# 3dhumangan/3DHumanGAN

Hardware: AMD Instinct MI355X
Metric: generator images/sec at 512^2 (higher is better)
Workload: dtype f32 in/out, f32 accumulate; contractions field f16x2 / synthesis f16x2 (x2 = f16 product + block-scaled fp6 cross terms, x3 = three f16/bf16 products); 1 GPU; BASELINE cfg 3: MAP3DBN512 generator-only forward, 512x512 out, 96x96 rays x 64 samples, hidden 256, batch 16/GPU, mixed, random-init weights, procedural SMPL-like pose; global_batch=16, parallelism=batch-sharded replicas x1 (no collective)

## Files before the change

### 3dhumangan_amd/csrc/geo_features.hip

```cpp
#include "common.hpp"

namespace {

constexpr int kThreads = 512;
constexpr int kPts = 4;
constexpr int kJoints = 24;
constexpr int kChunk = 64;
constexpr int kCand = 6;

typedef float f2 __attribute__((ext_vector_type(2)));
typedef float f4 __attribute__((ext_vector_type(4)));
typedef float f16v __attribute__((ext_vector_type(16)));
typedef unsigned u4 __attribute__((ext_vector_type(4)));
typedef int i4 __attribute__((ext_vector_type(4)));
typedef _Float16 half8 __attribute__((ext_vector_type(8)));
typedef _Float16 half2v __attribute__((ext_vector_type(2)));

__device__ __forceinline__ unsigned split2_f16(float a, float b, unsigned& lo) {
    const half2v h2 = __builtin_convertvector(f2{a, b}, half2v);
    lo = __builtin_bit_cast(unsigned, __builtin_convertvector(f2{a - (float)h2.x, b - (float)h2.y}, half2v));
    return __builtin_bit_cast(unsigned, h2);
}

__device__ __forceinline__ float sqdist_exact(float px, float py, float pz, float vx, float vy, float vz) {
    const float dx = __fsub_rn(px, vx), dy = __fsub_rn(py, vy), dz = __fsub_rn(pz, vz);
    return __fadd_rn(__fadd_rn(__fmul_rn(dx, dx), __fmul_rn(dy, dy)), __fmul_rn(dz, dz));
}

template <bool SORTED>
__device__ __forceinline__ void refine(const f4* vx4, const f4* vy4, const f4* vz4, const i4* ids4, int v4_begin, int v4_end,
                                       float px, float py, float pz, float& best, int& bi) {
#pragma clang loop unroll(disable)
    for (int v4 = v4_begin; v4 < v4_end; ++v4) {
        const f4 X = vx4[v4], Y = vy4[v4], Z = vz4[v4];
        const float d0 = sqdist_exact(px, py, pz, X.x, Y.x, Z.x);
        const float d1 = sqdist_exact(px, py, pz, X.y, Y.y, Z.y);
        const float d2 = sqdist_exact(px, py, pz, X.z, Y.z, Z.z);
        const float d3 = sqdist_exact(px, py, pz, X.w, Y.w, Z.w);
        if constexpr (SORTED) {
            const i4 I = ids4[v4];
            unsigned long long key = ((unsigned long long)__float_as_uint(best) << 32) | (unsigned)bi;
            const unsigned long long k0 = ((unsigned long long)__float_as_uint(d0) << 32) | (unsigned)I.x;
            const unsigned long long k1 = ((unsigned long long)__float_as_uint(d1) << 32) | (unsigned)I.y;
            const unsigned long long k2 = ((unsigned long long)__float_as_uint(d2) << 32) | (unsigned)I.z;
            const unsigned long long k3 = ((unsigned long long)__float_as_uint(d3) << 32) | (unsigned)I.w;
            key = k0 < key ? k0 : key;
            key = k1 < key ? k1 : key;
            key = k2 < key ? k2 : key;
            key = k3 < key ? k3 : key;
            best = __uint_as_float((unsigned)(key >> 32));
            bi = (int)(unsigned)key;
        } else {
            if (d0 < best) { best = d0; bi = v4 * 4 + 0; }
            if (d1 < best) { best = d1; bi = v4 * 4 + 1; }
            if (d2 < best) { best = d2; bi = v4 * 4 + 2; }
            if (d3 < best) { best = d3; bi = v4 * 4 + 3; }
        }
    }
}

template <bool FEATURES, bool SORTED>
__global__ __launch_bounds__(kThreads) void geo_features_kernel(
    const float* __restrict__ points, const float* __restrict__ joints, const float* __restrict__ vertices,
    const float* __restrict__ tpose, const float* __restrict__ vertex_ik, float* __restrict__ geo,
    int32_t* __restrict__ nn_index, int64_t N, int V, int Vpad, int geo_stride, int legacy_mode, int tile_S, int tile_Wr,
    int tiles_x, int tiles_y) {
    extern __shared__ __attribute__((aligned(16))) float smem[];
    float* vx = smem;
    float* vy = smem + Vpad;
    float* vz = smem + 2 * Vpad;
    int* vid = reinterpret_cast<int*>(smem + 3 * Vpad);
    float* jl = smem + (SORTED ? 4 : 3) * Vpad;
    unsigned* v2max_bits = reinterpret_cast<unsigned*>(jl + kJoints * 3);
    const int b = blockIdx.y;
    const int t = threadIdx.x;
    const float* __restrict__ vb = vertices + (int64_t)b * V * 3;
    const f4* __restrict__ ws = reinterpret_cast<const f4*>(vertices) + (int64_t)b * (Vpad + Vpad / kChunk);
    const f4* __restrict__ bounds = ws + Vpad;
    if (t == 0) *v2max_bits = 0u;
    __syncthreads();
    float v2 = 0.f;
    for (int i = t; i < Vpad; i += kThreads) {
        const bool ok = SORTED ? true : i < V;
        float x, y, z;
        if constexpr (SORTED) {
            const f4 q = ws[i];
            x = q.x; y = q.y; z = q.z;
            vid[i] = __float_as_int(q.w);
        } else {
            x = ok ? vb[i * 3 + 0] : 3.0e18f; y = ok ? vb[i * 3 + 1] : 3.0e18f; z = ok ? vb[i * 3 + 2] : 3.0e18f;
        }
        vx[i] = x; vy[i] = y; vz[i] = z;
        if (x < 1.0e18f) v2 = fmaxf(v2, x * x + y * y + z * z);
    }
    atomicMax(v2max_bits, __float_as_uint(v2));
    if (FEATURES && t < kJoints * 3) jl[t] = joints[(int64_t)b * kJoints * 3 + t];
    __syncthreads();
    const float v2max = __uint_as_float(*v2max_bits);

    const int lane = t & 63, m = lane & 31, hh = lane >> 5;
    const int64_t wave_id = (int64_t)blockIdx.x * (kThreads / 64) + (t >> 6);
    const int64_t wbase = wave_id * 256;
    int64_t tile_base = 0;
    bool tile_ok = true;
    if (tile_S > 0) {
        const int tiles_s = tile_S / 4;
        const int sz = (int)(wave_id % tiles_s);
        const int64_t pxy = wave_id / tiles_s;
        const int px_ = (int)(pxy % tiles_x), py_ = (int)(pxy / tiles_x);
        tile_ok = py_ < tiles_y;
        tile_base = (((int64_t)py_ * 8) * tile_Wr + px_ * 8) * tile_S + sz * 4;
    }
    auto point_of = [&](int i) -> int64_t {
        if (tile_S == 0) return wbase + i;
        if (!tile_ok) return N;
        const int ri = i >> 2;
        return tile_base + ((int64_t)(ri >> 3) * tile_Wr + (ri & 7)) * tile_S + (i & 3);
    };
    float px[kPts], py[kPts], pz[kPts], best[kPts];
    int bi[kPts];
#pragma unroll
    for (int k = 0; k < kPts; ++k) {
        const int64_t n = point_of((4 * hh + k) * 32 + m);
        const bool ok = n < N;
        const float* p = points + ((int64_t)b * N + (ok ? n : 0)) * 3;
        px[k] = p[0]; py[k] = p[1]; pz[k] = p[2];
        best[k] = 3.4e38f;
        bi[k] = 0;
    }
    const f4* vx4 = reinterpret_cast<const f4*>(vx);
    const f4* vy4 = reinterpret_cast<const f4*>(vy);
    const f4* vz4 = reinterpret_cast<const f4*>(vz);
    const i4* vid4 = reinterpret_cast<const i4*>(vid);

    half8 bfrag[8];
#pragma unroll
    for (int j = 0; j < 8; ++j) {
        const int k = j & 3;
        const float ox = __shfl_xor(px[k], 32, 64), oy = __shfl_xor(py[k], 32, 64), oz = __shfl_xor(pz[k], 32, 64);
        const bool own = (j >> 2) == hh;
        const float x = -2.f * (own ? px[k] : ox), y = -2.f * (own ? py[k] : oy), z = -2.f * (own ? pz[k] : oz);
        unsigned lo01, lo23;
        const unsigned hi01 = split2_f16(x, y, lo01), hi23 = split2_f16(z, 1.f, lo23);
        bfrag[j] = __builtin_bit_cast(half8, u4{hi01, hi23, hh ? 0u : lo01, hh ? 0u : lo23});
    }
    float run[kPts], tol[kPts], cval[kPts][kCand];
    float sk[kPts], sb[kPts];
    unsigned long long cid[kPts];
    int ncand[kPts];
#pragma unroll
    for (int k = 0; k < kPts; ++k) {
        const float p2 = px[k] * px[k] + py[k] * py[k] + pz[k] * pz[k];
        const float S = p2 + v2max;
        tol[k] = (S < 1.0e4f) ? 3.0517578e-5f * S : 3.0e38f;
        sb[k] = 3.f * tol[k] + p2;
        run[k] = 3.0e38f;
        sk[k] = 3.0e18f;
        cid[k] = 0ull;
        ncand[k] = 0;
#pragma unroll
        for (int q = 0; q < kCand; ++q) cval[k][q] = 3.4e38f;
    }
    const int n_chunks = Vpad / kChunk;
    int seed = -1;
    if constexpr (SORTED) {
        float sx = (px[0] + px[1]) + (px[2] + px[3]), sy = (py[0] + py[1]) + (py[2] + py[3]), sz = (pz[0] + pz[1]) + (pz[2] + pz[3]);
#pragma unroll
        for (int d = 32; d >= 1; d >>= 1) {
            sx += __shfl_xor(sx, d, 64); sy += __shfl_xor(sy, d, 64); sz += __shfl_xor(sz, d, 64);
        }
        sx *= 1.f / 256.f; sy *= 1.f / 256.f; sz *= 1.f / 256.f;
        float bd = 3.4e38f;
        int bc = 0;
        for (int c0 = lane; c0 < n_chunks; c0 += 64) {
            const f4 cb = bounds[c0];
            const float dx = sx - cb.x, dy = sy - cb.y, dz = sz - cb.z;
            const float d2 = dx * dx + dy * dy + dz * dz;
            if (d2 < bd) { bd = d2; bc = c0; }
        }
#pragma unroll
        for (int d = 32; d >= 1; d >>= 1) {
            const float od = __shfl_xor(bd, d, 64);
            const int oc = __shfl_xor(bc, d, 64);
            if (od < bd || (od == bd && oc < bc)) { bd = od; bc = oc; }
        }
        seed = __builtin_amdgcn_readfirstlane(bc);
    }
#pragma clang loop unroll(disable)
    for (int it = 0; it < n_chunks; ++it) {
        const int c = !SORTED ? it : it == 0 ? seed : (it <= seed ? it - 1 : it);
        if constexpr (SORTED) {
            const f4 cb = bounds[c];
            bool need = false;
#pragma unroll
            for (int k = 0; k < kPts; ++k) {
                const float dx = px[k] - cb.x, dy = py[k] - cb.y, dz = pz[k] - cb.z;
                const float d2 = dx * dx + dy * dy + dz * dz;
                const float reach = cb.w + sk[k];
                need |= d2 <= reach * reach;
            }
            if (__builtin_amdgcn_ballot_w64(need) == 0ull) continue;
        }
        float cmv[8];
#pragma unroll
        for (int j = 0; j < 8; ++j) cmv[j] = 3.4e38f;
#pragma unroll
        for (int tile = 0; tile < kChunk / 32; ++tile) {
            const int v = c * kChunk + tile * 32 + m;
            const bool real = v < V;
            const float x = real ? vx[v] : 0.f, y = real ? vy[v] : 0.f, z = real ? vz[v] : 0.f;
            const float w = real ? fmaf(z, z, fmaf(y, y, x * x)) : 6.0e4f;
            unsigned lo01, lo23;
            const unsigned hi01 = split2_f16(x, y, lo01), hi23 = split2_f16(z, w, lo23);
            const half8 afrag = __builtin_bit_cast(half8, hh ? u4{lo01, lo23, 0u, 0u} : u4{hi01, hi23, hi01, hi23});
#pragma unroll
            for (int j = 0; j < 8; ++j) {
                const f16v zero = {0.f, 0.f, 0.f, 0.f, 0.f, 0.f, 0.f, 0.f, 0.f, 0.f, 0.f, 0.f, 0.f, 0.f, 0.f, 0.f};
                const f16v d = __builtin_amdgcn_mfma_f32_32x32x16_f16(afrag, bfrag[j], zero, 0, 0, 0);
                float mn = cmv[j];
#pragma unroll
                for (int r = 0; r < 16; r += 2) mn = fminf(fminf(mn, d[r]), d[r + 1]);
                cmv[j] = mn;
            }
        }
        float cm[kPts];
#pragma unroll
        for (int k = 0; k < kPts; ++k) {
            const float lo_set = fminf(cmv[k], __shfl_xor(cmv[k], 32, 64));
            const float hi_set = fminf(cmv[4 + k], __shfl_xor(cmv[4 + k], 32, 64));
            cm[k] = hh ? hi_set : lo_set;
        }
#pragma unroll
        for (int k = 0; k < kPts; ++k) {
            if (cm[k] <= run[k] + tol[k]) {
#pragma unroll
                for (int q = 0; q < kCand - 1; ++q) cval[k][q] = cval[k][q + 1];
                cval[k][kCand - 1] = cm[k];
                cid[k] = (cid[k] << 8) | (unsigned long long)(c & 0xff);
                ++ncand[k];
                run[k] = fminf(run[k], cm[k]);
                if constexpr (SORTED)
                    sk[k] = __builtin_sqrtf(fmaxf(run[k] + sb[k], 0.f)) * 1.00001f;
            }
        }
    }
#pragma unroll
    for (int k = 0; k < kPts; ++k) {
        const bool overflow = ncand[k] > kCand && cval[k][0] <= run[k] + 2.f * tol[k];
        if (overflow) {
            refine<SORTED>(vx4, vy4, vz4, vid4, 0, Vpad / 4, px[k], py[k], pz[k], best[k], bi[k]);
        } else {
#pragma unroll
            for (int q = 0; q < kCand; ++q) {
                if (cval[k][q] <= run[k] + tol[k]) {
                    const int c = (int)((cid[k] >> (8 * (kCand - 1 - q))) & 0xffull);
                    refine<SORTED>(vx4, vy4, vz4, vid4, c * (kChunk / 4), (c + 1) * (kChunk / 4), px[k], py[k], pz[k], best[k], bi[k]);
                }
            }
        }
    }

#pragma unroll
    for (int k = 0; k < kPts; ++k) {
        const int64_t n = point_of((4 * hh + k) * 32 + m);
        if (n >= N) continue;
        const int idx = bi[k];
        if constexpr (!FEATURES) {
            nn_index[(int64_t)b * N + n] = idx;
            continue;
        }
        const float4* __restrict__ M = reinterpret_cast<const float4*>(vertex_ik + ((int64_t)b * V + idx) * 16);
        const float4 r0 = M[0], r1 = M[1], r2 = M[2];
        const float x = px[k], y = py[k], z = pz[k];
        const float cx = (r0.x * x + r0.y * y + r0.z * z + r0.w) / 2.f;
        const float cy = ((r1.x * x + r1.y * y + r1.z * z + r1.w) + 0.2f) / 2.f;
        const float cz = (r2.x * x + r2.y * y + r2.z * z + r2.w) / 1.3f;
        const float* __restrict__ tv = tpose + ((int64_t)b * V + idx) * 3;
        float* o = geo + ((int64_t)b * N + n) * geo_stride;
        float* oc = legacy_mode ? o + kJoints : o;
        float* oj = legacy_mode ? o : o + 3;
        oc[0] = cx; oc[1] = cy; oc[2] = cz;
#pragma unroll
        for (int j = 0; j < kJoints; ++j) {
            const float ax = x - jl[j * 3 + 0], ay = y - jl[j * 3 + 1], az = z - jl[j * 3 + 2];
            oj[j] = sqrtf(ax * ax + ay * ay + az * az) / 2.4f;
        }
        o[27] = tv[0]; o[28] = tv[1]; o[29] = tv[2] / 0.2f;
        o[30] = sqrtf(best[k]) / 1.3f;
        if (nn_index) nn_index[(int64_t)b * N + n] = idx;
    }
}

constexpr int kSortThreads = 1024;

__device__ __forceinline__ unsigned spread3(unsigned q) {
    q &= 0x3ffu;
    q = (q | (q << 16)) & 0x030000ffu;
    q = (q | (q << 8)) & 0x0300f00fu;
    q = (q | (q << 4)) & 0x030c30c3u;
    q = (q | (q << 2)) & 0x09249249u;
    return q;
}

__device__ __forceinline__ float wave_min(float v) {
#pragma unroll
    for (int d = 32; d >= 1; d >>= 1) v = fminf(v, __shfl_xor(v, d, 64));
    return v;
}
__device__ __forceinline__ float wave_max(float v) {
#pragma unroll
    for (int d = 32; d >= 1; d >>= 1) v = fmaxf(v, __shfl_xor(v, d, 64));
    return v;
}

__global__ __launch_bounds__(kSortThreads) void mesh_sort_kernel(const float* __restrict__ vertices, f4* __restrict__ ws, int V, int Vpad,
                                                                 int NP2) {
    extern __shared__ __attribute__((aligned(16))) unsigned long long keys[];
    __shared__ float box[6][kSortThreads / 64];
    const int b = blockIdx.x, t = threadIdx.x, lane = t & 63, wave = t >> 6;
    const float* __restrict__ vb = vertices + (int64_t)b * V * 3;
    f4* __restrict__ out = ws + (int64_t)b * (Vpad + Vpad / kChunk);
    float lo[3] = {3.0e38f, 3.0e38f, 3.0e38f}, hi[3] = {-3.0e38f, -3.0e38f, -3.0e38f};
    for (int i = t; i < V; i += kSortThreads)
#pragma unroll
        for (int a = 0; a < 3; ++a) {
            const float v = vb[i * 3 + a];
            lo[a] = fminf(lo[a], v); hi[a] = fmaxf(hi[a], v);
        }
#pragma unroll
    for (int a = 0; a < 3; ++a) {
        lo[a] = wave_min(lo[a]); hi[a] = wave_max(hi[a]);
        if (lane == 0) { box[a][wave] = lo[a]; box[3 + a][wave] = hi[a]; }
    }
    __syncthreads();
    float inv[3];
#pragma unroll
    for (int a = 0; a < 3; ++a) {
        float l = box[a][0], h = box[3 + a][0];
        for (int w = 1; w < kSortThreads / 64; ++w) { l = fminf(l, box[a][w]); h = fmaxf(h, box[3 + a][w]); }
        lo[a] = l;
        inv[a] = h > l ? 1023.f / (h - l) : 0.f;
    }
    for (int i = t; i < NP2; i += kSortThreads) {
        unsigned long long key = ~0ull;
        if (i < V) {
            unsigned code = 0;
#pragma unroll
            for (int a = 0; a < 3; ++a) {
                const float q = fminf(fmaxf((vb[i * 3 + a] - lo[a]) * inv[a], 0.f), 1023.f);
                code |= spread3((unsigned)q) << a;
            }
            key = ((unsigned long long)code << 32) | (unsigned)i;
        }
        keys[i] = key;
    }
    __syncthreads();
    for (int k = 2; k <= NP2; k <<= 1)
        for (int j = k >> 1; j > 0; j >>= 1) {
            for (int i = t; i < NP2; i += kSortThreads) {
                const int o = i ^ j;
                if (o > i) {
                    const unsigned long long a = keys[i], c = keys[o];
                    if ((a > c) == ((i & k) == 0)) { keys[i] = c; keys[o] = a; }
                }
            }
            __syncthreads();
        }
    for (int i = t; i < Vpad; i += kSortThreads) {
        if (i < V) {
            const int idx = (int)(unsigned)(keys[i] & 0xffffffffull);
            out[i] = f4{vb[idx * 3 + 0], vb[idx * 3 + 1], vb[idx * 3 + 2], __int_as_float(idx)};
        } else {
            out[i] = f4{3.0e18f, 3.0e18f, 3.0e18f, __int_as_float(0x7fffffff)};
        }
    }
    for (int c = wave; c < Vpad / kChunk; c += kSortThreads / 64) {
        const int i = c * kChunk + lane;
        const bool real = i < V;
        const int idx = real ? (int)(unsigned)(keys[i] & 0xffffffffull) : 0;
        const float x = vb[idx * 3 + 0], y = vb[idx * 3 + 1], z = vb[idx * 3 + 2];
        const float cx = 0.5f * (wave_min(real ? x : 3.0e38f) + wave_max(real ? x : -3.0e38f));
        const float cy = 0.5f * (wave_min(real ? y : 3.0e38f) + wave_max(real ? y : -3.0e38f));
        const float cz = 0.5f * (wave_min(real ? z : 3.0e38f) + wave_max(real ? z : -3.0e38f));
        const float dx = x - cx, dy = y - cy, dz = z - cz;
        const float r2 = wave_max(real ? dx * dx + dy * dy + dz * dz : 0.f);
        if (lane == 0) out[Vpad + c] = f4{cx, cy, cz, __builtin_sqrtf(r2) * 1.00001f + 1.0e-7f};
    }
}

int next_pow2(int v) {
    int p = 64;
    while (p < v) p <<= 1;
    return p;
}

}

static int geo_launch(bool features, bool sorted, const float* points, const float* joints, const float* vertices,
                      const float* tpose_vertices, const float* vertex_ik, float* geo, int32_t* nn_index,
                      int B, int64_t N, int V, int geo_stride, int legacy_mode, h3d_stream_t stream, int Hr = 0, int Wr = 0, int S = 0) {
    H3D_REQUIRE(B >= 0 && B <= 65535 && N >= 0, "h3d_geo_features / h3d_nearest_vertex: bad B=%d N=%lld", B, (long long)N);
    H3D_REQUIRE(V >= 1, "h3d_geo_features / h3d_nearest_vertex: V=%d", V);
    if (B == 0 || N == 0) return H3D_OK;
    const int Vpad = (V + kChunk - 1) / kChunk * kChunk;
    const size_t lds = sizeof(float) * ((sorted ? 4 : 3) * (size_t)Vpad + kJoints * 3 + 4);
    H3D_REQUIRE(lds <= 160 * 1024, "h3d_geo_features: mesh with V=%d vertices does not fit the 160 KB LDS", V);
    H3D_REQUIRE(!sorted || Vpad / kChunk <= 256, "h3d_geo_features: V=%d has more than 256 chunks", V);
    H3D_ALLOW_MAX_LDS((geo_features_kernel<true, false>));
    H3D_ALLOW_MAX_LDS((geo_features_kernel<false, false>));
    H3D_ALLOW_MAX_LDS((geo_features_kernel<true, true>));
    H3D_ALLOW_MAX_LDS((geo_features_kernel<false, true>));
    const int64_t per_block = (int64_t)kThreads * kPts;
    int64_t gx = (N + per_block - 1) / per_block;
    int tile_S = 0, tiles_x = 0, tiles_y = 0;
    if (S > 0 && Hr > 0 && Wr > 0 && (int64_t)Hr * Wr * S == N && Hr % 8 == 0 && Wr % 8 == 0 && S % 4 == 0) {
        tile_S = S; tiles_x = Wr / 8; tiles_y = Hr / 8;
        const int64_t waves = (int64_t)tiles_x * tiles_y * (S / 4);
        gx = (waves + kThreads / 64 - 1) / (kThreads / 64);
    }
    H3D_REQUIRE(gx < (int64_t(1) << 31), "h3d_geo_features: N too large");
    h3d::pre_launch();
    const dim3 grid((unsigned)gx, B), block(kThreads);
    hipStream_t st = static_cast<hipStream_t>(stream);
#define H3D_GEO_LAUNCH(F, S)                                                                                                    \
    hipLaunchKernelGGL((geo_features_kernel<F, S>), grid, block, lds, st, points, joints, vertices, tpose_vertices, vertex_ik, geo, \
                       nn_index, N, V, Vpad, geo_stride, legacy_mode, tile_S, Wr, tiles_x, tiles_y)
    if (features && sorted) H3D_GEO_LAUNCH(true, true);
    else if (features) H3D_GEO_LAUNCH(true, false);
    else if (sorted) H3D_GEO_LAUNCH(false, true);
    else H3D_GEO_LAUNCH(false, false);
#undef H3D_GEO_LAUNCH
    return h3d::launch_status(features ? "h3d_geo_features" : "h3d_nearest_vertex");
}

extern "C" int64_t h3d_mesh_sort_bytes(int B, int V) {
    if (B < 0 || V < 1) return -1;
    const int64_t Vpad = (V + kChunk - 1) / kChunk * kChunk;
    return (int64_t)B * (Vpad + Vpad / kChunk) * 16;
}

extern "C" int h3d_mesh_sort(const float* vertices, void* workspace, int B, int V, h3d_stream_t stream) {
    H3D_REQUIRE(vertices && workspace, "h3d_mesh_sort: null pointer");
    H3D_REQUIRE(B >= 0 && B <= 65535 && V >= 1, "h3d_mesh_sort: bad B=%d V=%d", B, V);
    H3D_REQUIRE(h3d::aligned16(workspace), "h3d_mesh_sort: the workspace must be 16-byte aligned");
    if (B == 0) return H3D_OK;
    const int Vpad = (V + kChunk - 1) / kChunk * kChunk, NP2 = next_pow2(V);
    H3D_REQUIRE((size_t)NP2 * 8 <= 128 * 1024, "h3d_mesh_sort: V=%d does not fit the LDS sort (max 16384)", V);
    H3D_ALLOW_MAX_LDS(mesh_sort_kernel);
    h3d::pre_launch();
    hipLaunchKernelGGL(mesh_sort_kernel, dim3(B), dim3(kSortThreads), (size_t)NP2 * 8, static_cast<hipStream_t>(stream), vertices,
                       static_cast<f4*>(workspace), V, Vpad, NP2);
    return h3d::launch_status("h3d_mesh_sort");
}

extern "C" int h3d_geo_features(const float* points, const float* joints, const float* vertices,
                                const float* tpose_vertices, const float* vertex_ik, float* geo, int32_t* nn_index,
                                int B, int64_t N, int V, int geo_stride, int legacy_mode, h3d_stream_t stream) {
    H3D_REQUIRE(points && joints && vertices && tpose_vertices && vertex_ik && geo, "h3d_geo_features: null pointer");
    H3D_REQUIRE(geo_stride >= 31, "h3d_geo_features: geo_stride=%d must be >= 31", geo_stride);
    H3D_REQUIRE(h3d::aligned16(vertex_ik), "h3d_geo_features: vertex_ik must be 16-byte aligned");
    return geo_launch(true, false, points, joints, vertices, tpose_vertices, vertex_ik, geo, nn_index, B, N, V, geo_stride, legacy_mode, stream);
}

extern "C" int h3d_nearest_vertex(const float* points, const float* vertices, int32_t* nn_index, int B, int64_t N, int V,
                                  h3d_stream_t stream) {
    H3D_REQUIRE(points && vertices && nn_index, "h3d_nearest_vertex: null pointer");
    return geo_launch(false, false, points, nullptr, vertices, nullptr, nullptr, nullptr, nn_index, B, N, V, 31, 0, stream);
}

extern "C" int h3d_geo_features_sorted(const float* points, const float* joints, const void* sorted_mesh,
                                       const float* tpose_vertices, const float* vertex_ik, float* geo, int32_t* nn_index,
                                       int B, int64_t N, int V, int geo_stride, int legacy_mode, h3d_stream_t stream) {
    H3D_REQUIRE(points && joints && sorted_mesh && tpose_vertices && vertex_ik && geo, "h3d_geo_features_sorted: null pointer");
    H3D_REQUIRE(geo_stride >= 31, "h3d_geo_features_sorted: geo_stride=%d must be >= 31", geo_stride);
    H3D_REQUIRE(h3d::aligned16(vertex_ik) && h3d::aligned16(sorted_mesh), "h3d_geo_features_sorted: vertex_ik / sorted_mesh must be 16-byte aligned");
    return geo_launch(true, true, points, joints, static_cast<const float*>(sorted_mesh), tpose_vertices, vertex_ik, geo, nn_index, B, N, V,
                      geo_stride, legacy_mode, stream);
}

extern "C" int h3d_nearest_vertex_sorted_rays(const float* points, const void* sorted_mesh, int32_t* nn_index, int B, int Hr, int Wr,
                                              int S, int V, h3d_stream_t stream) {
    H3D_REQUIRE(points && sorted_mesh && nn_index, "h3d_nearest_vertex_sorted_rays: null pointer");
    H3D_REQUIRE(h3d::aligned16(sorted_mesh), "h3d_nearest_vertex_sorted_rays: sorted_mesh must be 16-byte aligned");
    H3D_REQUIRE(Hr >= 1 && Wr >= 1 && S >= 1, "h3d_nearest_vertex_sorted_rays: bad grid %dx%dx%d", Hr, Wr, S);
    return geo_launch(false, true, points, nullptr, static_cast<const float*>(sorted_mesh), nullptr, nullptr, nullptr, nn_index, B,
                      (int64_t)Hr * Wr * S, V, 31, 0, stream, Hr, Wr, S);
}

extern "C" int h3d_nearest_vertex_sorted(const float* points, const void* sorted_mesh, int32_t* nn_index, int B, int64_t N, int V,
                                         h3d_stream_t stream) {
    H3D_REQUIRE(points && sorted_mesh && nn_index, "h3d_nearest_vertex_sorted: null pointer");
    H3D_REQUIRE(h3d::aligned16(sorted_mesh), "h3d_nearest_vertex_sorted: sorted_mesh must be 16-byte aligned");
    return geo_launch(false, true, points, nullptr, static_cast<const float*>(sorted_mesh), nullptr, nullptr, nullptr, nn_index, B, N, V, 31, 0,
                      stream);
}
```

Before: 354.3 images/s.

## Add persistent ray-tiled nearest-vertex kernel with wave-level chunk culling

Moves the per-wave nearest-vertex search into a shared helper and adds a persistent kernel for the ray-tiled path. The kernel launches one block per compute unit, loads each batch's sorted mesh and chunk bounds into LDS once, and loops over 8x8x4 ray tiles. The sorted search no longer walks every chunk in order. It builds a wave bounding sphere, ballots 64 chunk bounds at a time, and visits only chunks within reach, which cuts per-chunk bound checks and repeated mesh loads from global memory. The cost is more LDS for the bounds and a grid-stride persistent schedule that may balance load unevenly.

Result: no change. 354.5 images/s, median of 3 (+0.1%).

```diff
diff --git a/3dhumangan_amd/csrc/geo_features.hip b/3dhumangan_amd/csrc/geo_features.hip
--- a/3dhumangan_amd/csrc/geo_features.hip
+++ b/3dhumangan_amd/csrc/geo_features.hip
@@ -20,6 +20,21 @@
     const half2v h2 = __builtin_convertvector(f2{a, b}, half2v);
     lo = __builtin_bit_cast(unsigned, __builtin_convertvector(f2{a - (float)h2.x, b - (float)h2.y}, half2v));
     return __builtin_bit_cast(unsigned, h2);
+}
+
+__device__ __forceinline__ float wave_min(float v) {
+#pragma unroll
+    for (int d = 32; d >= 1; d >>= 1) v = fminf(v, __shfl_xor(v, d, 64));
+    return v;
+}
+__device__ __forceinline__ float wave_max(float v) {
+#pragma unroll
+    for (int d = 32; d >= 1; d >>= 1) v = fmaxf(v, __shfl_xor(v, d, 64));
+    return v;
+}
+
+__device__ __forceinline__ float uniform(float v) {
+    return __uint_as_float(__builtin_amdgcn_readfirstlane(__float_as_uint(v)));
 }
 
 __device__ __forceinline__ float sqdist_exact(float px, float py, float pz, float vx, float vy, float vz) {
@@ -59,12 +74,184 @@
     }
 }
 
+template <bool SORTED>
+__device__ __forceinline__ void search_wave(const float* vx, const float* vy, const float* vz, const int* vid, const f4* bounds, int V,
+                                            int Vpad, float v2max, int lane, const float (&px)[kPts], const float (&py)[kPts],
+                                            const float (&pz)[kPts], float (&best)[kPts], int (&bi)[kPts]) {
+    const int m = lane & 31, hh = lane >> 5;
+    const f4* vx4 = reinterpret_cast<const f4*>(vx);
+    const f4* vy4 = reinterpret_cast<const f4*>(vy);
+    const f4* vz4 = reinterpret_cast<const f4*>(vz);
+    const i4* vid4 = reinterpret_cast<const i4*>(vid);
+    half8 bfrag[8];
+#pragma unroll
+    for (int j = 0; j < 8; ++j) {
+        const int k = j & 3;
+        const float ox = __shfl_xor(px[k], 32, 64), oy = __shfl_xor(py[k], 32, 64), oz = __shfl_xor(pz[k], 32, 64);
+        const bool own = (j >> 2) == hh;
+        const float x = -2.f * (own ? px[k] : ox), y = -2.f * (own ? py[k] : oy), z = -2.f * (own ? pz[k] : oz);
+        unsigned lo01, lo23;
+        const unsigned hi01 = split2_f16(x, y, lo01), hi23 = split2_f16(z, 1.f, lo23);
+        bfrag[j] = __builtin_bit_cast(half8, u4{hi01, hi23, hh ? 0u : lo01, hh ? 0u : lo23});
+    }
+    float run[kPts], tol[kPts], cval[kPts][kCand];
+    float sk[kPts];
+    unsigned long long cid[kPts];
+    int ncand[kPts];
+#pragma unroll
+    for (int k = 0; k < kPts; ++k) {
+        const float p2 = px[k] * px[k] + py[k] * py[k] + pz[k] * pz[k];
+        const float S = p2 + v2max;
+        tol[k] = (S < 1.0e4f) ? 3.0517578e-5f * S : 3.0e38f;
+        run[k] = 3.0e38f;
+        sk[k] = 3.0e18f;
+        cid[k] = 0ull;
+        ncand[k] = 0;
+#pragma unroll
+        for (int q = 0; q < kCand; ++q) cval[k][q] = 3.4e38f;
+    }
+    const int n_chunks = Vpad / kChunk;
+    int seed = -1;
+    float gx = 0.f, gy = 0.f, gz = 0.f, gr = 0.f;
+    if constexpr (SORTED) {
+        gx = (px[0] + px[1]) + (px[2] + px[3]); gy = (py[0] + py[1]) + (py[2] + py[3]); gz = (pz[0] + pz[1]) + (pz[2] + pz[3]);
+#pragma unroll
+        for (int d = 32; d >= 1; d >>= 1) {
+            gx += __shfl_xor(gx, d, 64); gy += __shfl_xor(gy, d, 64); gz += __shfl_xor(gz, d, 64);
+        }
+        gx = uniform(gx * (1.f / 256.f)); gy = uniform(gy * (1.f / 256.f)); gz = uniform(gz * (1.f / 256.f));
+        float bd = 3.4e38f;
+        int bc = 0;
+        for (int c0 = lane; c0 < n_chunks; c0 += 64) {
+            const f4 cb = bounds[c0];
+            const float dx = gx - cb.x, dy = gy - cb.y, dz = gz - cb.z;
+            const float d2 = dx * dx + dy * dy + dz * dz;
+            if (d2 < bd) { bd = d2; bc = c0; }
+        }
+#pragma unroll
+        for (int d = 32; d >= 1; d >>= 1) {
+            const float od = __shfl_xor(bd, d, 64);
+            const int oc = __shfl_xor(bc, d, 64);
+            if (od < bd || (od == bd && oc < bc)) { bd = od; bc = oc; }
+        }
+        seed = __builtin_amdgcn_readfirstlane(bc);
+#pragma unroll
+        for (int k = 0; k < kPts; ++k) {
+            const float dx = px[k] - gx, dy = py[k] - gy, dz = pz[k] - gz;
+            gr = fmaxf(gr, dx * dx + dy * dy + dz * dz);
+        }
+        gr = uniform(__builtin_sqrtf(wave_max(gr)) * 1.00001f);
+    }
+    unsigned long long pend = 0ull;
+    int base = -64;
+#pragma clang loop unroll(disable)
+    for (int it = 0;; ++it) {
+        int c = it;
+        if constexpr (!SORTED) {
+            if (it >= n_chunks) break;
+        } else {
+            if (it == 0) {
+                c = seed;
+            } else {
+                while (pend == 0ull && (base += 64) < n_chunks) {
+                    const float smax = uniform(wave_max(fmaxf(fmaxf(sk[0], sk[1]), fmaxf(sk[2], sk[3]))));
+                    const int ci = base + lane;
+                    bool keep = false;
+                    if (ci < n_chunks) {
+                        const f4 cb = bounds[ci];
+                        const float dx = gx - cb.x, dy = gy - cb.y, dz = gz - cb.z;
+                        const float reach = (gr + cb.w) + smax;
+                        keep = !(dx * dx + dy * dy + dz * dz > reach * reach * 1.00002f);
+                    }
+                    pend = __builtin_amdgcn_ballot_w64(keep);
+                }
+                if (pend == 0ull) break;
+                c = base + __builtin_ctzll(pend);
+                pend &= pend - 1ull;
+                if (c == seed) continue;
+            }
+            const f4 cb = bounds[c];
+            bool need = false;
+#pragma unroll
+            for (int k = 0; k < kPts; ++k) {
+                const float dx = px[k] - cb.x, dy = py[k] - cb.y, dz = pz[k] - cb.z;
+                const float d2 = dx * dx + dy * dy + dz * dz;
+                const float reach = cb.w + sk[k];
+                need |= d2 <= reach * reach;
+            }
+            if (__builtin_amdgcn_ballot_w64(need) == 0ull) continue;
+        }
+        float cmv[8];
+#pragma unroll
+        for (int j = 0; j < 8; ++j) cmv[j] = 3.4e38f;
+#pragma unroll
+        for (int tile = 0; tile < kChunk / 32; ++tile) {
+            const int v = c * kChunk + tile * 32 + m;
+            const bool real = v < V;
+            const float x = real ? vx[v] : 0.f, y = real ? vy[v] : 0.f, z = real ? vz[v] : 0.f;
+            const float w = real ? fmaf(z, z, fmaf(y, y, x * x)) : 6.0e4f;
+            unsigned lo01, lo23;
+            const unsigned hi01 = split2_f16(x, y, lo01), hi23 = split2_f16(z, w, lo23);
+            u4 abits = hh ? u4{lo01, lo23, 0u, 0u} : u4{hi01, hi23, hi01, hi23};
+#pragma unroll
+            for (int j = 0; j < 8; ++j) {
+                const f16v zero = {0.f, 0.f, 0.f, 0.f, 0.f, 0.f, 0.f, 0.f, 0.f, 0.f, 0.f, 0.f, 0.f, 0.f, 0.f, 0.f};
+                const f16v d = __builtin_amdgcn_mfma_f32_32x32x16_f16(__builtin_bit_cast(half8, abits), bfrag[j], zero, 0, 0, 0);
+                float mn = cmv[j];
+#pragma unroll
+                for (int r = 0; r < 16; r += 2) mn = fminf(fminf(mn, d[r]), d[r + 1]);
+                cmv[j] = mn;
+                if (j == 3) asm volatile("" : "+v"(abits), "+v"(cmv[0]), "+v"(cmv[1]), "+v"(cmv[2]), "+v"(cmv[3]));
+            }
+        }
+        float cm[kPts];
+#pragma unroll
+        for (int k = 0; k < kPts; ++k) {
+            const float lo_set = fminf(cmv[k], __shfl_xor(cmv[k], 32, 64));
+            const float hi_set = fminf(cmv[4 + k], __shfl_xor(cmv[4 + k], 32, 64));
+            cm[k] = hh ? hi_set : lo_set;
+        }
+#pragma unroll
+        for (int k = 0; k < kPts; ++k) {
+            if (cm[k] <= run[k] + tol[k]) {
+#pragma unroll
+                for (int q = 0; q < kCand - 1; ++q) cval[k][q] = cval[k][q + 1];
+                cval[k][kCand - 1] = cm[k];
+                cid[k] = (cid[k] << 8) | (unsigned long long)(c & 0xff);
+                ++ncand[k];
+                run[k] = fminf(run[k], cm[k]);
+                if constexpr (SORTED) {
+                    const float sb = 3.f * tol[k] + (px[k] * px[k] + py[k] * py[k] + pz[k] * pz[k]);
+                    sk[k] = __builtin_sqrtf(fmaxf(run[k] + sb, 0.f)) * 1.00001f;
+                }
+            }
+        }
+    }
+#pragma unroll
+    for (int k = 0; k < kPts; ++k) {
+        best[k] = 3.4e38f;
+        bi[k] = 0;
+        const bool overflow = ncand[k] > kCand && cval[k][0] <= run[k] + 2.f * tol[k];
+        if (overflow) {
+            refine<SORTED>(vx4, vy4, vz4, vid4, 0, Vpad / 4, px[k], py[k], pz[k], best[k], bi[k]);
+        } else {
+#pragma unroll
+            for (int q = 0; q < kCand; ++q) {
+                if (cval[k][q] <= run[k] + tol[k]) {
+                    const int c = (int)((cid[k] >> (8 * (kCand - 1 - q))) & 0xffull);
+                    refine<SORTED>(vx4, vy4, vz4, vid4, c * (kChunk / 4), (c + 1) * (kChunk / 4), px[k], py[k], pz[k], best[k], bi[k]);
+                }
+            }
+        }
+    }
+
+}
+
 template <bool FEATURES, bool SORTED>
 __global__ __launch_bounds__(kThreads) void geo_features_kernel(
     const float* __restrict__ points, const float* __restrict__ joints, const float* __restrict__ vertices,
     const float* __restrict__ tpose, const float* __restrict__ vertex_ik, float* __restrict__ geo,
-    int32_t* __restrict__ nn_index, int64_t N, int V, int Vpad, int geo_stride, int legacy_mode, int tile_S, int tile_Wr,
-    int tiles_x, int tiles_y) {
+    int32_t* __restrict__ nn_index, int64_t N, int V, int Vpad, int geo_stride, int legacy_mode) {
     extern __shared__ __attribute__((aligned(16))) float smem[];
     float* vx = smem;
     float* vy = smem + Vpad;
@@ -99,24 +286,8 @@
     const float v2max = __uint_as_float(*v2max_bits);
 
     const int lane = t & 63, m = lane & 31, hh = lane >> 5;
-    const int64_t wave_id = (int64_t)blockIdx.x * (kThreads / 64) + (t >> 6);
-    const int64_t wbase = wave_id * 256;
-    int64_t tile_base = 0;
-    bool tile_ok = true;
-    if (tile_S > 0) {
-        const int tiles_s = tile_S / 4;
-        const int sz = (int)(wave_id % tiles_s);
-        const int64_t pxy = wave_id / tiles_s;
-        const int px_ = (int)(pxy % tiles_x), py_ = (int)(pxy / tiles_x);
-        tile_ok = py_ < tiles_y;
-        tile_base = (((int64_t)py_ * 8) * tile_Wr + px_ * 8) * tile_S + sz * 4;
-    }
-    auto point_of = [&](int i) -> int64_t {
-        if (tile_S == 0) return wbase + i;
-        if (!tile_ok) return N;
-        const int ri = i >> 2;
-        return tile_base + ((int64_t)(ri >> 3) * tile_Wr + (ri & 7)) * tile_S + (i & 3);
-    };
+    const int64_t wbase = ((int64_t)blockIdx.x * (kThreads / 64) + (t >> 6)) * 256;
+    auto point_of = [&](int i) -> int64_t { return wbase + i; };
     float px[kPts], py[kPts], pz[kPts], best[kPts];
     int bi[kPts];
 #pragma unroll
@@ -125,140 +296,8 @@
         const bool ok = n < N;
         const float* p = points + ((int64_t)b * N + (ok ? n : 0)) * 3;
         px[k] = p[0]; py[k] = p[1]; pz[k] = p[2];
-        best[k] = 3.4e38f;
-        bi[k] = 0;
-    }
-    const f4* vx4 = reinterpret_cast<const f4*>(vx);
-    const f4* vy4 = reinterpret_cast<const f4*>(vy);
-    const f4* vz4 = reinterpret_cast<const f4*>(vz);
-    const i4* vid4 = reinterpret_cast<const i4*>(vid);
-
-    half8 bfrag[8];
-#pragma unroll
-    for (int j = 0; j < 8; ++j) {
-        const int k = j & 3;
-        const float ox = __shfl_xor(px[k], 32, 64), oy = __shfl_xor(py[k], 32, 64), oz = __shfl_xor(pz[k], 32, 64);
-        const bool own = (j >> 2) == hh;
-        const float x = -2.f * (own ? px[k] : ox), y = -2.f * (own ? py[k] : oy), z = -2.f * (own ? pz[k] : oz);
-        unsigned lo01, lo23;
-        const unsigned hi01 = split2_f16(x, y, lo01), hi23 = split2_f16(z, 1.f, lo23);
-        bfrag[j] = __builtin_bit_cast(half8, u4{hi01, hi23, hh ? 0u : lo01, hh ? 0u : lo23});
-    }
-    float run[kPts], tol[kPts], cval[kPts][kCand];
-    float sk[kPts], sb[kPts];
-    unsigned long long cid[kPts];
-    int ncand[kPts];
-#pragma unroll
-    for (int k = 0; k < kPts; ++k) {
-        const float p2 = px[k] * px[k] + py[k] * py[k] + pz[k] * pz[k];
-        const float S = p2 + v2max;
-        tol[k] = (S < 1.0e4f) ? 3.0517578e-5f * S : 3.0e38f;
-        sb[k] = 3.f * tol[k] + p2;
-        run[k] = 3.0e38f;
-        sk[k] = 3.0e18f;
-        cid[k] = 0ull;
-        ncand[k] = 0;
-#pragma unroll
-        for (int q = 0; q < kCand; ++q) cval[k][q] = 3.4e38f;
-    }
-    const int n_chunks = Vpad / kChunk;
-    int seed = -1;
-    if constexpr (SORTED) {
-        float sx = (px[0] + px[1]) + (px[2] + px[3]), sy = (py[0] + py[1]) + (py[2] + py[3]), sz = (pz[0] + pz[1]) + (pz[2] + pz[3]);
-#pragma unroll
-        for (int d = 32; d >= 1; d >>= 1) {
-            sx += __shfl_xor(sx, d, 64); sy += __shfl_xor(sy, d, 64); sz += __shfl_xor(sz, d, 64);
-        }
-        sx *= 1.f / 256.f; sy *= 1.f / 256.f; sz *= 1.f / 256.f;
-        float bd = 3.4e38f;
-        int bc = 0;
-        for (int c0 = lane; c0 < n_chunks; c0 += 64) {
-            const f4 cb = bounds[c0];
-            const float dx = sx - cb.x, dy = sy - cb.y, dz = sz - cb.z;
-            const float d2 = dx * dx + dy * dy + dz * dz;
-            if (d2 < bd) { bd = d2; bc = c0; }
-        }
-#pragma unroll
-        for (int d = 32; d >= 1; d >>= 1) {
-            const float od = __shfl_xor(bd, d, 64);
-            const int oc = __shfl_xor(bc, d, 64);
-            if (od < bd || (od == bd && oc < bc)) { bd = od; bc = oc; }
-        }
-        seed = __builtin_amdgcn_readfirstlane(bc);
-    }
-#pragma clang loop unroll(disable)
-    for (int it = 0; it < n_chunks; ++it) {
-        const int c = !SORTED ? it : it == 0 ? seed : (it <= seed ? it - 1 : it);
-        if constexpr (SORTED) {
-            const f4 cb = bounds[c];
-            bool need = false;
-#pragma unroll
-            for (int k = 0; k < kPts; ++k) {
-                const float dx = px[k] - cb.x, dy = py[k] - cb.y, dz = pz[k] - cb.z;
-                const float d2 = dx * dx + dy * dy + dz * dz;
-                const float reach = cb.w + sk[k];
-                need |= d2 <= reach * reach;
-            }
-            if (__builtin_amdgcn_ballot_w64(need) == 0ull) continue;
-        }
-        float cmv[8];
-#pragma unroll
-        for (int j = 0; j < 8; ++j) cmv[j] = 3.4e38f;
-#pragma unroll
-        for (int tile = 0; tile < kChunk / 32; ++tile) {
-            const int v = c * kChunk + tile * 32 + m;
-            const bool real = v < V;
-            const float x = real ? vx[v] : 0.f, y = real ? vy[v] : 0.f, z = real ? vz[v] : 0.f;
-            const float w = real ? fmaf(z, z, fmaf(y, y, x * x)) : 6.0e4f;
-            unsigned lo01, lo23;
-            const unsigned hi01 = split2_f16(x, y, lo01), hi23 = split2_f16(z, w, lo23);
-            const half8 afrag = __builtin_bit_cast(half8, hh ? u4{lo01, lo23, 0u, 0u} : u4{hi01, hi23, hi01, hi23});
-#pragma unroll
-            for (int j = 0; j < 8; ++j) {
-                const f16v zero = {0.f, 0.f, 0.f, 0.f, 0.f, 0.f, 0.f, 0.f, 0.f, 0.f, 0.f, 0.f, 0.f, 0.f, 0.f, 0.f};
-                const f16v d = __builtin_amdgcn_mfma_f32_32x32x16_f16(afrag, bfrag[j], zero, 0, 0, 0);
-                float mn = cmv[j];
-#pragma unroll
-                for (int r = 0; r < 16; r += 2) mn = fminf(fminf(mn, d[r]), d[r + 1]);
-                cmv[j] = mn;
-            }
-        }
-        float cm[kPts];
-#pragma unroll
-        for (int k = 0; k < kPts; ++k) {
-            const float lo_set = fminf(cmv[k], __shfl_xor(cmv[k], 32, 64));
-            const float hi_set = fminf(cmv[4 + k], __shfl_xor(cmv[4 + k], 32, 64));
-            cm[k] = hh ? hi_set : lo_set;
-        }
-#pragma unroll
-        for (int k = 0; k < kPts; ++k) {
-            if (cm[k] <= run[k] + tol[k]) {
-#pragma unroll
-                for (int q = 0; q < kCand - 1; ++q) cval[k][q] = cval[k][q + 1];
-                cval[k][kCand - 1] = cm[k];
-                cid[k] = (cid[k] << 8) | (unsigned long long)(c & 0xff);
-                ++ncand[k];
-                run[k] = fminf(run[k], cm[k]);
-                if constexpr (SORTED)
-                    sk[k] = __builtin_sqrtf(fmaxf(run[k] + sb[k], 0.f)) * 1.00001f;
-            }
-        }
-    }
-#pragma unroll
-    for (int k = 0; k < kPts; ++k) {
-        const bool overflow = ncand[k] > kCand && cval[k][0] <= run[k] + 2.f * tol[k];
-        if (overflow) {
-            refine<SORTED>(vx4, vy4, vz4, vid4, 0, Vpad / 4, px[k], py[k], pz[k], best[k], bi[k]);
-        } else {
-#pragma unroll
-            for (int q = 0; q < kCand; ++q) {
-                if (cval[k][q] <= run[k] + tol[k]) {
-                    const int c = (int)((cid[k] >> (8 * (kCand - 1 - q))) & 0xffull);
-                    refine<SORTED>(vx4, vy4, vz4, vid4, c * (kChunk / 4), (c + 1) * (kChunk / 4), px[k], py[k], pz[k], best[k], bi[k]);
-                }
-            }
-        }
-    }
+    }
+    search_wave<SORTED>(vx, vy, vz, vid, bounds, V, Vpad, v2max, lane, px, py, pz, best, bi);
 
 #pragma unroll
     for (int k = 0; k < kPts; ++k) {
@@ -291,6 +330,62 @@
     }
 }
 
+__global__ __launch_bounds__(kThreads) void nearest_rays_kernel(const float* __restrict__ points, const f4* __restrict__ sorted_mesh,
+                                                                int32_t* __restrict__ nn_index, int B, int V, int Vpad, int Wr, int S,
+                                                                int tiles_x, int tiles_y) {
+    extern __shared__ __attribute__((aligned(16))) float smem[];
+    const int n_chunks = Vpad / kChunk;
+    float* vx = smem;
+    float* vy = smem + Vpad;
+    float* vz = smem + 2 * Vpad;
+    int* vid = reinterpret_cast<int*>(smem + 3 * Vpad);
+    f4* bounds = reinterpret_cast<f4*>(smem + 4 * Vpad);
+    unsigned* v2max_bits = reinterpret_cast<unsigned*>(smem + 4 * Vpad + 4 * n_chunks);
+    const int t = threadIdx.x, lane = t & 63, m = lane & 31, hh = lane >> 5;
+    const int tiles_s = S / 4;
+    const int64_t T = (int64_t)tiles_x * tiles_y * tiles_s;
+    const int64_t N = (int64_t)tiles_y * 8 * Wr * S;
+    const int64_t n_slots = (int64_t)gridDim.x * (kThreads / 64);
+    const int64_t slot = (int64_t)blockIdx.x * (kThreads / 64) + __builtin_amdgcn_readfirstlane(t >> 6);
+    const int lane_off = ((hh * 4) * Wr + (m >> 2)) * S + (m & 3);
+    for (int b = 0; b < B; ++b) {
+        int64_t w = (slot - (int64_t)b * T) % n_slots;
+        if (w < 0) w += n_slots;
+        if (!__syncthreads_or(w < T)) continue;
+        if (t == 0) *v2max_bits = 0u;
+        __syncthreads();
+        const f4* __restrict__ ws = sorted_mesh + (int64_t)b * (Vpad + n_chunks);
+        float v2 = 0.f;
+        for (int i = t; i < Vpad; i += kThreads) {
+            const f4 q = ws[i];
+            vx[i] = q.x; vy[i] = q.y; vz[i] = q.z;
+            vid[i] = __float_as_int(q.w);
+            if (q.x < 1.0e18f) v2 = fmaxf(v2, q.x * q.x + q.y * q.y + q.z * q.z);
+        }
+        for (int i = t; i < n_chunks; i += kThreads) bounds[i] = ws[Vpad + i];
+        atomicMax(v2max_bits, __float_as_uint(v2));
+        __syncthreads();
+        const float v2max = __uint_as_float(*v2max_bits);
+        for (; w < T; w += n_slots) {
+            const int sz = (int)(w % tiles_s);
+            const int64_t pxy = w / tiles_s;
+            const int tx = (int)(pxy % tiles_x), ty = (int)(pxy / tiles_x);
+            const int64_t tile_base = (((int64_t)ty * 8) * Wr + tx * 8) * S + sz * 4;
+            const int64_t n0 = (int64_t)b * N + tile_base + lane_off;
+            float px[kPts], py[kPts], pz[kPts], best[kPts];
+            int bi[kPts];
+#pragma unroll
+            for (int k = 0; k < kPts; ++k) {
+                const float* p = points + (n0 + (int64_t)k * Wr * S) * 3;
+                px[k] = p[0]; py[k] = p[1]; pz[k] = p[2];
+            }
+            search_wave<true>(vx, vy, vz, vid, bounds, V, Vpad, v2max, lane, px, py, pz, best, bi);
+#pragma unroll
+            for (int k = 0; k < kPts; ++k) nn_index[n0 + (int64_t)k * Wr * S] = bi[k];
+        }
+    }
+}
+
 constexpr int kSortThreads = 1024;
 
 __device__ __forceinline__ unsigned spread3(unsigned q) {
@@ -300,17 +395,6 @@
     q = (q | (q << 4)) & 0x030c30c3u;
     q = (q | (q << 2)) & 0x09249249u;
     return q;
-}
-
-__device__ __forceinline__ float wave_min(float v) {
-#pragma unroll
-    for (int d = 32; d >= 1; d >>= 1) v = fminf(v, __shfl_xor(v, d, 64));
-    return v;
-}
-__device__ __forceinline__ float wave_max(float v) {
-#pragma unroll
-    for (int d = 32; d >= 1; d >>= 1) v = fmaxf(v, __shfl_xor(v, d, 64));
-    return v;
 }
 
 __global__ __launch_bounds__(kSortThreads) void mesh_sort_kernel(const float* __restrict__ vertices, f4* __restrict__ ws, int V, int Vpad,
@@ -398,7 +482,7 @@
 
 static int geo_launch(bool features, bool sorted, const float* points, const float* joints, const float* vertices,
                       const float* tpose_vertices, const float* vertex_ik, float* geo, int32_t* nn_index,
-                      int B, int64_t N, int V, int geo_stride, int legacy_mode, h3d_stream_t stream, int Hr = 0, int Wr = 0, int S = 0) {
+                      int B, int64_t N, int V, int geo_stride, int legacy_mode, h3d_stream_t stream) {
     H3D_REQUIRE(B >= 0 && B <= 65535 && N >= 0, "h3d_geo_features / h3d_nearest_vertex: bad B=%d N=%lld", B, (long long)N);
     H3D_REQUIRE(V >= 1, "h3d_geo_features / h3d_nearest_vertex: V=%d", V);
     if (B == 0 || N == 0) return H3D_OK;
@@ -411,20 +495,14 @@
     H3D_ALLOW_MAX_LDS((geo_features_kernel<true, true>));
     H3D_ALLOW_MAX_LDS((geo_features_kernel<false, true>));
     const int64_t per_block = (int64_t)kThreads * kPts;
-    int64_t gx = (N + per_block - 1) / per_block;
-    int tile_S = 0, tiles_x = 0, tiles_y = 0;
-    if (S > 0 && Hr > 0 && Wr > 0 && (int64_t)Hr * Wr * S == N && Hr % 8 == 0 && Wr % 8 == 0 && S % 4 == 0) {
-        tile_S = S; tiles_x = Wr / 8; tiles_y = Hr / 8;
-        const int64_t waves = (int64_t)tiles_x * tiles_y * (S / 4);
-        gx = (waves + kThreads / 64 - 1) / (kThreads / 64);
-    }
+    const int64_t gx = (N + per_block - 1) / per_block;
     H3D_REQUIRE(gx < (int64_t(1) << 31), "h3d_geo_features: N too large");
     h3d::pre_launch();
     const dim3 grid((unsigned)gx, B), block(kThreads);
     hipStream_t st = static_cast<hipStream_t>(stream);
 #define H3D_GEO_LAUNCH(F, S)                                                                                                    \
     hipLaunchKernelGGL((geo_features_kernel<F, S>), grid, block, lds, st, points, joints, vertices, tpose_vertices, vertex_ik, geo, \
-                       nn_index, N, V, Vpad, geo_stride, legacy_mode, tile_S, Wr, tiles_x, tiles_y)
+                       nn_index, N, V, Vpad, geo_stride, legacy_mode)
     if (features && sorted) H3D_GEO_LAUNCH(true, true);
     else if (features) H3D_GEO_LAUNCH(true, false);
     else if (sorted) H3D_GEO_LAUNCH(false, true);
@@ -483,8 +561,24 @@
     H3D_REQUIRE(points && sorted_mesh && nn_index, "h3d_nearest_vertex_sorted_rays: null pointer");
     H3D_REQUIRE(h3d::aligned16(sorted_mesh), "h3d_nearest_vertex_sorted_rays: sorted_mesh must be 16-byte aligned");
     H3D_REQUIRE(Hr >= 1 && Wr >= 1 && S >= 1, "h3d_nearest_vertex_sorted_rays: bad grid %dx%dx%d", Hr, Wr, S);
-    return geo_launch(false, true, points, nullptr, static_cast<const float*>(sorted_mesh), nullptr, nullptr, nullptr, nn_index, B,
-                      (int64_t)Hr * Wr * S, V, 31, 0, stream, Hr, Wr, S);
+    H3D_REQUIRE(B >= 0 && B <= 65535 && V >= 1, "h3d_nearest_vertex_sorted_rays: bad B=%d V=%d", B, V);
+    const int Vpad = (V + kChunk - 1) / kChunk * kChunk, n_chunks = Vpad / kChunk;
+    const size_t lds = sizeof(float) * (4 * (size_t)Vpad + 4 * (size_t)n_chunks + 4);
+    if (Hr % 8 != 0 || Wr % 8 != 0 || S % 4 != 0 || lds > 160 * 1024 || (int64_t)Hr * Wr * S * 3 >= (int64_t(1) << 31))
+        return geo_launch(false, true, points, nullptr, static_cast<const float*>(sorted_mesh), nullptr, nullptr, nullptr, nn_index, B,
+                          (int64_t)Hr * Wr * S, V, 31, 0, stream);
+    if (B == 0) return H3D_OK;
+    H3D_REQUIRE(n_chunks <= 256, "h3d_nearest_vertex_sorted_rays: V=%d has more than 256 chunks", V);
+    H3D_ALLOW_MAX_LDS(nearest_rays_kernel);
+    const int tiles_x = Wr / 8, tiles_y = Hr / 8;
+    const int64_t waves = (int64_t)B * tiles_x * tiles_y * (S / 4);
+    const int64_t groups = (waves + kThreads / 64 - 1) / (kThreads / 64);
+    const int cus = h3d::compute_units();
+    h3d::pre_launch();
+    hipLaunchKernelGGL(nearest_rays_kernel, dim3((unsigned)(groups < cus ? groups : cus)), dim3(kThreads), lds,
+                       static_cast<hipStream_t>(stream), points, static_cast<const f4*>(sorted_mesh), nn_index, B, V, Vpad, Wr, S, tiles_x,
+                       tiles_y);
+    return h3d::launch_status("h3d_nearest_vertex_sorted_rays");
 }
 
 extern "C" int h3d_nearest_vertex_sorted(const float* points, const void* sorted_mesh, int32_t* nn_index, int B, int64_t N, int V,
```
